# duyhominhnguyen/conan-fgw

Hardware: AMD Instinct MI355X
Metric: molecules/s (K=5 conformers) (higher is better)
Workload: dtype f32

## Files before the change

### conan-fgw_amd/_lib.py

```python
from __future__ import annotations

import ctypes
import os
import subprocess

import torch

_HERE = os.path.dirname(os.path.abspath(__file__))
_SO = os.path.join(_HERE, "libconan_fgw_hip.so")
_LIB = None
ABI_VERSION = 6

c_int, c_float, c_void_p, c_ll = ctypes.c_int, ctypes.c_float, ctypes.c_void_p, ctypes.c_longlong


class FgwParams(ctypes.Structure):
    _fields_ = [("alpha", c_float), ("epsilon", c_float), ("max_iter", c_int), ("tol", c_float), ("inner_tol", c_float),
                ("num_iter_max", c_int), ("stop_thr", c_float), ("fixed_structure", c_int), ("fixed_features", c_int),
                ("warmstart", c_int), ("loss_fun", c_int), ("cs_small_int", c_int)]


class BatchLayout(ctypes.Structure):
    _fields_ = [(n, c_int) for n in ("B", "K", "num_graphs", "num_atoms", "num_bond_edges", "max_nodes", "x_dim", "ea_dim")] + \
               [(n, c_ll) for n in ("off_atom_off", "off_bond_off", "off_z", "off_pos", "off_x", "off_bsrc", "off_bdst", "off_battr", "off_y", "bytes")]


class WgradJob(ctypes.Structure):
    _fields_ = [("ws", c_void_p), ("dW", c_void_p), ("dbias", c_void_p), ("M", c_int), ("K", c_int), ("N", c_int), ("slices", c_int)]


class WgradSlabJob(ctypes.Structure):
    _fields_ = [("g", c_void_p), ("x", c_void_p), ("m_dev", c_void_p), ("ws", c_void_p), ("M", c_int), ("K", c_int), ("N", c_int), ("slices", c_int)]


_P = c_void_p
SIGNATURES = {
    "conan_abi_version": (c_int, []),
    "conan_collate_layout": (c_int, [c_int, c_int, _P, _P, c_int, c_int, ctypes.POINTER(BatchLayout)]),
    "conan_collate_pack": (c_int, [ctypes.POINTER(BatchLayout), _P, _P, _P, _P, _P, _P, _P, _P, _P]),
    "conan_collate_unpack": (c_int, [_P, ctypes.POINTER(BatchLayout), _P, _P, _P, _P, _P, _P, _P, _P, _P, _P, _P]),
    "conan_graph_ptr_from_batch": (c_int, [_P, c_int, c_int, _P, _P]),
    "conan_radius_graph_csr": (c_int, [_P, _P, c_int, c_int, c_float, c_int, c_int, _P, _P, _P, _P, _P, _P]),
    "conan_csr_transpose": (c_int, [_P, c_int, c_int, _P, _P, _P, _P, _P, _P]),
    "conan_edge_pairs": (c_int, [_P, _P, _P, _P, _P, c_int, _P, _P, _P, _P, _P, _P, _P, _P]),
    "conan_edge_index_i64": (c_int, [_P, _P, c_int, _P, _P]),
    "conan_embedding_fwd": (c_int, [_P, _P, c_int, c_int, c_int, _P, _P]),
    "conan_onehot_rows": (c_int, [_P, c_int, c_int, c_int, _P, _P]),
    "conan_embedding_bwd_ws": (c_ll, [c_int, c_int, c_int]),
    "conan_embedding_bwd": (c_int, [_P, _P, c_int, c_int, c_int, c_int, _P, _P, _P]),
    "conan_linear_fwd": (c_int, [_P, _P, _P, _P, c_int, c_int, c_int, c_int, c_int, _P, _P, _P]),
    "conan_linear_multi_fwd": (c_int, [_P, _P, _P, c_int, c_int, c_int, c_int, c_int, _P, _P, _P, _P]),
    "conan_linear_sum_fwd": (c_int, [_P, _P, _P, c_int, c_int, _P, _P, c_int, c_int, _P, _P, _P]),
    "conan_ssp_bwd": (c_int, [_P, _P, c_int, c_int, _P, _P, _P]),
    "conan_linear_wgrad_ws": (c_ll, [c_int, c_int, c_int]),
    "conan_linear_wgrad": (c_int, [_P, _P, c_int, c_int, c_int, _P, _P, _P, _P, _P]),
    "conan_bond_graph_csr": (c_int, [_P, c_int, c_int, _P, _P, _P, _P, _P, _P, _P, _P]),
    "conan_gat_edge_vec": (c_int, [_P, _P, c_int, c_int, _P, _P]),
    "conan_gat_edge_vec_bwd": (c_int, [_P, _P, _P, c_int, c_int, _P, _P, _P]),
    "conan_gat_node_alpha": (c_int, [_P, _P, _P, c_int, c_int, _P, _P, _P]),
    "conan_gat_aggregate_fwd": (c_int, [_P, _P, _P, _P, _P, _P, _P, c_int, _P, _P, c_float, c_int, c_int, _P, _P, _P, _P]),
    "conan_gat_bwd_ws": (c_ll, [c_int, c_int, c_int, c_int]),
    "conan_gat_aggregate_bwd": (c_int, [_P] * 15 + [c_int, _P, c_float, c_int, c_int, c_int, _P, _P, _P, _P]),
    "conan_linear_act_fwd": (c_int, [_P, _P, _P, c_int, c_int, c_int, c_int, _P, _P, _P, _P]),
    "conan_unary_fwd": (c_int, [_P, c_ll, c_int, _P, _P]),
    "conan_unary_bwd": (c_int, [_P, _P, c_ll, c_int, _P, _P]),
    "conan_zero_tail": (c_int, [_P, _P, c_int, c_int, _P]),
    "conan_rbf_wgrad": (c_int, [_P, _P, c_int, _P, c_int, c_float, c_int, _P, _P, _P, _P, _P]),
    "conan_wgrad_batchable": (c_int, [c_int, c_int]),
    "conan_linear_wgrad_scaled": (c_int, [_P, _P, c_int, c_int, c_int, _P, _P, _P, _P, _P, _P]),
    "conan_linear_wgrad_slabs": (c_int, [_P, _P, c_int, c_int, c_int, _P, _P, _P]),
    "conan_rbf_wgrad_slabs": (c_int, [_P, _P, c_int, _P, c_int, c_float, c_int, _P, _P, _P]),
    "conan_wgrad_reduce_batch": (c_int, [ctypes.POINTER(WgradJob), c_int, _P]),
    "conan_linear_wgrad_slabs_batch": (c_int, [ctypes.POINTER(WgradSlabJob), c_int, _P]),
    "conan_filter_bwd_supported": (c_int, [c_int, c_int]),
    "conan_filter_bwd_slices": (c_int, [c_int]),
    "conan_filter_bwd_ws": (c_ll, [c_int, c_int, c_int]),
    "conan_filter_bwd": (c_int, [_P, _P, _P, c_int, _P, c_int, c_float, _P, c_int, _P, _P, _P, _P, _P, _P]),
# ... 160 lines not shown
```

### conan-fgw_amd/csrc/graph.hip

```cpp
#include "common.h"

namespace {

__global__ void k_graph_ptr(const int64_t *__restrict__ batch, int n, int G, int *__restrict__ ptr) {
    int i = blockIdx.x * blockDim.x + threadIdx.x;
    if (i >= n) return;
    long long cur = batch[i];
    long long prev = i == 0 ? -1 : batch[i - 1];
    for (long long g = prev + 1; g <= cur && g < G; ++g) ptr[g] = i;
    if (i == n - 1)
        for (long long g = cur + 1; g <= G; ++g) ptr[g] = n;
}
__global__ void k_graph_ptr_empty(int G, int *ptr) {
    int g = blockIdx.x * blockDim.x + threadIdx.x;
    if (g <= G) ptr[g] = 0;
}

__device__ __forceinline__ float dist2_rn(float ax, float ay, float az, float bx, float by, float bz) {
    float dx = __fsub_rn(ax, bx), dy = __fsub_rn(ay, by), dz = __fsub_rn(az, bz);
    return __fadd_rn(__fadd_rn(__fmul_rn(dx, dx), __fmul_rn(dy, dy)), __fmul_rn(dz, dz));
}

constexpr int RG_THREADS = 128;
constexpr int RG_MAX_LDS_ATOMS = 2048;
// ... 38 lines not shown
constexpr int SCAN_LDS_MAX = 36 * 1024;
__global__ void __launch_bounds__(1024) k_exclusive_scan_lds(const int *__restrict__ in, int n, int *__restrict__ out) {
    extern __shared__ int sdat[];
    int *wsum = sdat + n;
    const int t = threadIdx.x, lane = t & 63, wave = t >> 6;
    for (int i0 = t; i0 < n; i0 += 4 * 1024) {
        int v[4];
#pragma unroll
        for (int u = 0; u < 4; ++u) { const int i = i0 + u * 1024; v[u] = in[i < n ? i : n - 1]; }
#pragma unroll
        for (int u = 0; u < 4; ++u) { const int i = i0 + u * 1024; if (i < n) sdat[i] = v[u]; }
    }
    __syncthreads();
    const int chunk = ((n + 1023) / 1024) | 1;
    const int b = min(t * chunk, n), e = min(b + chunk, n);
    int s = 0;
    for (int i = b; i < e; ++i) s += sdat[i];
    int inc = s;
#pragma unroll
    for (int o = 1; o < 64; o <<= 1) { const int u = __shfl_up(inc, o, 64); if (lane >= o) inc += u; }
    if (lane == 63) wsum[wave] = inc;
    __syncthreads();
    int woff = 0, total = 0;
#pragma unroll
    for (int w = 0; w < 16; ++w) { const int x = wsum[w]; if (w < wave) woff += x; total += x; }
    int run = woff + inc - s;
    for (int i = b; i < e; ++i) { const int x = sdat[i]; sdat[i] = run; run += x; }
    __syncthreads();
    for (int i = t; i < n; i += 1024) out[i] = sdat[i];
    if (t == 0) out[n] = total;
}

constexpr int SCAN_THREADS = 1024;
__global__ void __launch_bounds__(SCAN_THREADS) k_exclusive_scan(const int *__restrict__ in, int n, int *__restrict__ out) {
    __shared__ int wsum[SCAN_THREADS / 64];
    const int t = threadIdx.x, lane = t & 63, wave = t >> 6;
    const int chunk = (n + SCAN_THREADS - 1) / SCAN_THREADS;
    const int b = t * chunk, e = min(b + chunk, n);
    constexpr int MAXC = 32;
    int v[MAXC];
    int s = 0;
    if (chunk <= MAXC) {
#pragma unroll
        for (int k = 0; k < MAXC; ++k) { v[k] = (b + k < e) ? in[b + k] : 0; }
#pragma unroll
        for (int k = 0; k < MAXC; ++k) s += v[k];
    } else {
        for (int i = b; i < e; ++i) s += in[i];
    }
    int inc = s;
#pragma unroll
    for (int o = 1; o < 64; o <<= 1) { const int u = __shfl_up(inc, o, 64); if (lane >= o) inc += u; }
    if (lane == 63) wsum[wave] = inc;
    __syncthreads();
    int woff = 0, total = 0;
#pragma unroll
    for (int w = 0; w < SCAN_THREADS / 64; ++w) { const int x = wsum[w]; if (w < wave) woff += x; total += x; }
    int run = woff + inc - s;
    if (chunk <= MAXC) {
#pragma unroll
        for (int k = 0; k < MAXC; ++k) if (b + k < e) { out[b + k] = run; run += v[k]; }
    } else {
        for (int i = b; i < e; ++i) { const int x = in[i]; out[i] = run; run += x; }
    }
    if (t == 0) out[n] = total;
}

static void launch_exclusive_scan(const int *in, int n, int *out, hipStream_t s) {
    if (n > 0 && n <= SCAN_LDS_MAX) {
        const size_t lds = (size_t)(n + 16) * sizeof(int);
        if (lds > 64 * 1024)
            (void)hipFuncSetAttribute(reinterpret_cast<const void *>(&k_exclusive_scan_lds), hipFuncAttributeMaxDynamicSharedMemorySize, (int)lds);
        k_exclusive_scan_lds<<<1, 1024, lds, s>>>(in, n, out);
    } else {
        k_exclusive_scan<<<1, SCAN_THREADS, 0, s>>>(in, n, out);
    }
}

constexpr int SB_THREADS = 256;
constexpr int SB_ITEMS = 16;
__global__ void __launch_bounds__(SB_THREADS) k_scan_block_sums(const int *__restrict__ in, int n, int *__restrict__ bsum) {
    __shared__ int red[SB_THREADS / 64];
    const int base = blockIdx.x * SB_THREADS * SB_ITEMS + threadIdx.x * SB_ITEMS;
    int s = 0;
#pragma unroll
    for (int u = 0; u < SB_ITEMS; ++u) s += (base + u < n) ? in[base + u] : 0;
    s = wave_sum(s);
    if ((threadIdx.x & 63) == 0) red[threadIdx.x >> 6] = s;
    __syncthreads();
    if (threadIdx.x == 0) bsum[blockIdx.x] = red[0] + red[1] + red[2] + red[3];
}
__global__ void __launch_bounds__(SB_THREADS) k_scan_block_apply(const int *__restrict__ in, int n, const int *__restrict__ boff,
                                                                 int nblocks, int *__restrict__ out) {
    __shared__ int part[SB_THREADS];
    const int t = threadIdx.x;
    const int base = blockIdx.x * SB_THREADS * SB_ITEMS + t * SB_ITEMS;
    int v[SB_ITEMS], s = 0;
#pragma unroll
    for (int u = 0; u < SB_ITEMS; ++u) { v[u] = (base + u < n) ? in[base + u] : 0; s += v[u]; }
    part[t] = s;
    __syncthreads();
    for (int o = 1; o < SB_THREADS; o <<= 1) {
        const int a = t >= o ? part[t - o] : 0;
        __syncthreads();
        part[t] += a;
        __syncthreads();
    }
    int run = boff[blockIdx.x] + (t == 0 ? 0 : part[t - 1]);
#pragma unroll
    for (int u = 0; u < SB_ITEMS; ++u) { if (base + u < n) out[base + u] = run; run += v[u]; }
    if (blockIdx.x == nblocks - 1 && t == SB_THREADS - 1) out[n] = boff[nblocks];
}
static void scan_large(const int *in, int n, int *out, int *ws, hipStream_t s) {
    const int per = SB_THREADS * SB_ITEMS;
    const int nblocks = (n + per - 1) / per;
    int *bsum = ws, *boff = ws + nblocks + 1;
    k_scan_block_sums<<<nblocks, SB_THREADS, 0, s>>>(in, n, bsum);
    launch_exclusive_scan(bsum, nblocks, boff, s);
    k_scan_block_apply<<<nblocks, SB_THREADS, 0, s>>>(in, n, boff, nblocks, out);
}

constexpr int TR_THREADS = 1024;
__global__ void __launch_bounds__(TR_THREADS) k_transpose_graph(const int *__restrict__ gptr, const int *__restrict__ rowptr,
                                                                const int *__restrict__ col, int num_atoms,
                                                                int *__restrict__ t_rowptr, int *__restrict__ t_eid) {
    const int g = blockIdx.x;
    const int lo = gptr[g], hi = gptr[g + 1];
    if (g == gridDim.x - 1 && threadIdx.x == 0) t_rowptr[num_atoms] = rowptr[num_atoms];
    if (hi <= lo) return;
    const int e0 = rowptr[lo], e1 = rowptr[hi];
    const int steps = (e1 - e0 + 63) >> 6;
    const int lane = threadIdx.x & 63, wave = threadIdx.x >> 6;
    const unsigned long long below = (1ull << lane) - 1ull;
    constexpr int TR_REG = 18;
    if (steps <= TR_REG) {
        int cv[TR_REG];
#pragma unroll
        for (int s = 0; s < TR_REG; ++s) {
            const int e = e0 + s * 64 + lane;
            cv[s] = (s < steps && e < e1) ? col[e] : 0x7fffffff;
        }
        for (int j = lo + wave; j < hi; j += TR_THREADS / 64) {
            int less = 0;
#pragma unroll
            for (int s = 0; s < TR_REG; ++s) less += __popcll(__ballot(cv[s] < j));
            int base = e0 + less;
            if (lane == 0) t_rowptr[j] = base;
#pragma unroll
            for (int s = 0; s < TR_REG; ++s) {
                const bool hit = cv[s] == j;
                const unsigned long long m = __ballot(hit);
                if (hit) t_eid[base + __popcll(m & below)] = e0 + s * 64 + lane;
                base += __popcll(m);
            }
        }
        return;
    }
    constexpr int TR_LDS = 4096;
    __shared__ int sc[TR_LDS];
    if (steps * 64 <= TR_LDS) {
        for (int q = threadIdx.x; q < steps * 64; q += TR_THREADS) sc[q] = (e0 + q < e1) ? col[e0 + q] : 0x7fffffff;
        __syncthreads();
        for (int j = lo + wave; j < hi; j += TR_THREADS / 64) {
            int less = 0;
            for (int s = 0; s < steps; ++s) less += __popcll(__ballot(sc[s * 64 + lane] < j));
            int base = e0 + less;
            if (lane == 0) t_rowptr[j] = base;
            for (int s = 0; s < steps; ++s) {
                const bool hit = sc[s * 64 + lane] == j;
                const unsigned long long m = __ballot(hit);
                if (hit) t_eid[base + __popcll(m & below)] = e0 + s * 64 + lane;
                base += __popcll(m);
            }
        }
        return;
    }
    for (int j = lo + wave; j < hi; j += TR_THREADS / 64) {
        int less = 0;
        for (int s = 0; s < steps; ++s) {
            const int e = e0 + s * 64 + lane;
            less += __popcll(__ballot(e < e1 && col[e] < j));
        }
        int base = e0 + less;
        if (lane == 0) t_rowptr[j] = base;
        for (int s = 0; s < steps; ++s) {
            const int e = e0 + s * 64 + lane;
            const bool hit = e < e1 && col[e] == j;
            const unsigned long long m = __ballot(hit);
            if (hit) t_eid[base + __popcll(m & below)] = e;
            base += __popcll(m);
        }
    }
}

__device__ __forceinline__ int find_edge(const int *__restrict__ rowptr, const int *__restrict__ col, int target, int source) {
    int lo = rowptr[target], hi = rowptr[target + 1] - 1;
    while (lo <= hi) {
        const int mid = (lo + hi) >> 1;
        const int c = col[mid];
        if (c == source) return mid;
        if (c < source) lo = mid + 1; else hi = mid - 1;
    }
    return -1;
}
__global__ void k_pair_flag(const int *__restrict__ rowptr, const int *__restrict__ col, const int *__restrict__ tgt,
                            const int *__restrict__ ne_dev, int max_edges, int *__restrict__ flag) {
    const int E = min(*ne_dev, max_edges);
    for (int e = blockIdx.x * blockDim.x + threadIdx.x; e < max_edges; e += gridDim.x * blockDim.x) {
        int f = 0;
        if (e < E) {
            const int s = col[e], t = tgt[e];
            f = (s <= t) ? 1 : (find_edge(rowptr, col, s, t) < 0 ? 1 : 0);
        }
        flag[e] = f;
    }
}
__global__ void k_pair_fill(const int *__restrict__ rowptr, const int *__restrict__ col, const int *__restrict__ tgt, const float *__restrict__ dist,
                            const int *__restrict__ ne_dev, int max_edges, const int *__restrict__ flag, const int *__restrict__ pidx,
                            int *__restrict__ pid, int *__restrict__ pe0, int *__restrict__ pe1, float *__restrict__ pdist) {
    const int E = min(*ne_dev, max_edges);
    for (int e = blockIdx.x * blockDim.x + threadIdx.x; e < E; e += gridDim.x * blockDim.x) {
        const int s = col[e], t = tgt[e];
        const int rev = (s == t) ? -1 : find_edge(rowptr, col, s, t);
        if (flag[e]) {
            const int p = pidx[e];
            pid[e] = p; pe0[p] = e; pe1[p] = rev; pdist[p] = dist[e];
        } else {
            pid[e] = pidx[rev];
        }
    }
}

__global__ void k_edge_index(const int *__restrict__ col, const int *__restrict__ tgt, int E, int64_t *__restrict__ ei) {
    int e = blockIdx.x * blockDim.x + threadIdx.x;
    if (e < E) { ei[e] = col[e]; ei[(size_t)E + e] = tgt[e]; }
}


__global__ void k_bond_count(const int64_t *__restrict__ ei, int E, int n, int *__restrict__ deg_t, int *__restrict__ deg_s) {
    for (int e = blockIdx.x * blockDim.x + threadIdx.x; e < E; e += gridDim.x * blockDim.x) {
        const int s = (int)ei[e], t = (int)ei[(size_t)E + e];
        if (s == t || s < 0 || t < 0 || s >= n || t >= n) continue;
        atomicAdd(&deg_t[t], 1);
        atomicAdd(&deg_s[s], 1);
    }
}
__global__ void k_bond_fill_t(const int64_t *__restrict__ ei, int E, int n, const int *__restrict__ rowptr, int *__restrict__ cursor,
                              int *__restrict__ col, int *__restrict__ eid) {
    for (int e = blockIdx.x * blockDim.x + threadIdx.x; e < E; e += gridDim.x * blockDim.x) {
        const int s = (int)ei[e], t = (int)ei[(size_t)E + e];
        if (s == t || s < 0 || t < 0 || s >= n || t >= n) continue;
        const int p = rowptr[t] + atomicAdd(&cursor[t], 1);
        col[p] = s; eid[p] = e;
    }
}
__global__ void k_rows_sort2(const int *__restrict__ rowptr, int n, int *__restrict__ key, int *__restrict__ val) {
    for (int i = blockIdx.x * blockDim.x + threadIdx.x; i < n; i += gridDim.x * blockDim.x) {
        const int a = rowptr[i], b = rowptr[i + 1];
        for (int p = a + 1; p < b; ++p) {
            const int k = key[p], v = val[p];
            int q = p - 1;
            while (q >= a && (key[q] > k || (key[q] == k && val[q] > v))) { key[q + 1] = key[q]; val[q + 1] = val[q]; --q; }
            key[q + 1] = k; val[q + 1] = v;
        }
    }
// ... 30 lines not shown
                           int loop, int *deg_ws, int *rowptr, int *col, int *tgt, float *dist, void *stream) {
    if (!pos || !graph_ptr || !deg_ws || !rowptr || !col || !tgt || !dist || num_atoms < 0 || num_graphs <= 0 || cap <= 0)
        return CONAN_E_BADARG;
    hipStream_t s = as_stream(stream);
    const float r2 = r * r;
    k_radius<0><<<num_graphs, RG_THREADS, 0, s>>>(pos, graph_ptr, r2, cap, loop, deg_ws, nullptr, nullptr, nullptr, nullptr);
    launch_exclusive_scan(deg_ws, num_atoms, rowptr, s);
    k_radius<1><<<num_graphs, RG_THREADS, 0, s>>>(pos, graph_ptr, r2, cap, loop, nullptr, rowptr, col, tgt, dist);
    CONAN_LAUNCH_CHECK();
    return CONAN_OK;
}

int conan_csr_transpose(const int *graph_ptr, int num_graphs, int num_atoms, const int *rowptr, const int *col,
                        int *deg_ws, int *t_rowptr, int *t_eid, void *stream) {
    if (!graph_ptr || !rowptr || !col || !t_rowptr || !t_eid || num_graphs <= 0) return CONAN_E_BADARG;
    hipStream_t s = as_stream(stream);
    (void)deg_ws;
    k_transpose_graph<<<num_graphs, TR_THREADS, 0, s>>>(graph_ptr, rowptr, col, num_atoms, t_rowptr, t_eid);
    CONAN_LAUNCH_CHECK();
    return CONAN_OK;
}

int conan_edge_pairs(const int *rowptr, const int *col, const int *tgt, const float *dist, const int *num_edges_dev, int max_edges,
                     int *flag_ws, int *pidx_ws, int *scan_ws, int *pid, int *pair_e0, int *pair_e1, float *pair_dist, void *stream) {
    if (!rowptr || !col || !tgt || !dist || !num_edges_dev || !flag_ws || !pidx_ws || !scan_ws || !pid || !pair_e0 || !pair_e1 || !pair_dist ||
        max_edges <= 0)
        return CONAN_E_BADARG;
    hipStream_t s = as_stream(stream);
    int blocks = (max_edges + 255) / 256;
    if (blocks > 4096) blocks = 4096;
    k_pair_flag<<<blocks, 256, 0, s>>>(rowptr, col, tgt, num_edges_dev, max_edges, flag_ws);
    scan_large(flag_ws, max_edges, pidx_ws, scan_ws, s);
    k_pair_fill<<<blocks, 256, 0, s>>>(rowptr, col, tgt, dist, num_edges_dev, max_edges, flag_ws, pidx_ws, pid, pair_e0, pair_e1, pair_dist);
    CONAN_LAUNCH_CHECK();
    return CONAN_OK;
}

int conan_bond_graph_csr(const int64_t *edge_index, int num_edges, int num_nodes, int *ws, int *rowptr, int *col, int *eid,
                         int *t_rowptr, int *t_pos, int *t_tgt, void *stream) {
    if (num_edges < 0 || num_nodes <= 0 || !ws || !rowptr || !t_rowptr || (num_edges && (!edge_index || !col || !eid || !t_pos || !t_tgt)))
        return CONAN_E_BADARG;
    hipStream_t s = as_stream(stream);
    int *deg_t = ws, *deg_s = ws + (num_nodes + 1);
    if (hipMemsetAsync(ws, 0, sizeof(int) * 2 * (size_t)(num_nodes + 1), s) != hipSuccess) return CONAN_E_LAUNCH;
    const int eb = num_edges ? (num_edges + 255) / 256 : 1, nb = (num_nodes + 255) / 256;
    if (num_edges) k_bond_count<<<eb, 256, 0, s>>>(edge_index, num_edges, num_nodes, deg_t, deg_s);
    launch_exclusive_scan(deg_t, num_nodes, rowptr, s);
    launch_exclusive_scan(deg_s, num_nodes, t_rowptr, s);
    if (num_edges) {
        if (hipMemsetAsync(ws, 0, sizeof(int) * 2 * (size_t)(num_nodes + 1), s) != hipSuccess) return CONAN_E_LAUNCH;
        k_bond_fill_t<<<eb, 256, 0, s>>>(edge_index, num_edges, num_nodes, rowptr, deg_t, col, eid);
        k_rows_sort2<<<nb, 256, 0, s>>>(rowptr, num_nodes, col, eid);
        k_bond_fill_s<<<nb, 256, 0, s>>>(rowptr, col, num_nodes, t_rowptr, deg_s, t_pos, t_tgt);
        k_rows_sort2<<<nb, 256, 0, s>>>(t_rowptr, num_nodes, t_pos, t_tgt);
    }
    CONAN_LAUNCH_CHECK();
    return CONAN_OK;
}

int conan_edge_index_i64(const int *col, const int *tgt, int num_edges, int64_t *edge_index, void *stream) {
    if (num_edges < 0 || (num_edges && (!col || !tgt || !edge_index))) return CONAN_E_BADARG;
    if (num_edges == 0) return CONAN_OK;
    k_edge_index<<<(num_edges + 255) / 256, 256, 0, as_stream(stream)>>>(col, tgt, num_edges, edge_index);
    CONAN_LAUNCH_CHECK();
    return CONAN_OK;
}
// ... 3 lines not shown
```

### conan-fgw_amd/ops.py

```python
from __future__ import annotations

import ctypes
from typing import Optional

import torch
from torch import Tensor

from ._lib import FgwParams, call, lib, ptr, stream_ptr

f32, i32, i64 = torch.float32, torch.int32, torch.int64


def _c(t: Tensor) -> Tensor:
    return t if t.is_contiguous() else t.contiguous()


class RadiusGraph:

    def __init__(self, pos: Tensor, graph_ptr: Tensor, num_graphs: int, cutoff: float, max_num_neighbors: int, loop: bool = False):
        pos = _c(pos)
        if pos.dtype != f32:
            raise RuntimeError("pos must be float32")
        n = pos.shape[0]
        dev = pos.device
        self.num_atoms, self.num_graphs, self.graph_ptr = n, num_graphs, graph_ptr
        self.cutoff, self.cap, self.loop = float(cutoff), int(max_num_neighbors), bool(loop)
        self.max_edges = max(1, n * (self.cap if self.loop else self.cap + 1))
        self.rowptr = torch.empty(n + 1, dtype=i32, device=dev)
        self.col = torch.empty(self.max_edges, dtype=i32, device=dev)
        self.tgt = torch.empty(self.max_edges, dtype=i32, device=dev)
        self.dist = torch.empty(self.max_edges, dtype=f32, device=dev)
        self._deg = torch.empty(n + 1, dtype=i32, device=dev)
        call("conan_radius_graph_csr", ptr(pos), ptr(graph_ptr, i32), n, num_graphs, self.cutoff, self.cap, int(self.loop),
             ptr(self._deg), ptr(self.rowptr), ptr(self.col), ptr(self.tgt), ptr(self.dist), stream_ptr())
        self.num_edges_dev = self.rowptr[n:]
        self._num_edges: Optional[int] = None
        self._t_rowptr = self._t_eid = None
        self.pid = None

    @property
    def num_edges(self) -> int:
        if self._num_edges is None:
            self._num_edges = int(self.num_edges_dev.item())
        return self._num_edges

    def transpose(self):
        if self._t_rowptr is None:
            dev = self.rowptr.device
            self._t_rowptr = torch.empty(self.num_atoms + 1, dtype=i32, device=dev)
            self._t_eid = torch.empty(self.max_edges, dtype=i32, device=dev)
            call("conan_csr_transpose", ptr(self.graph_ptr), self.num_graphs, self.num_atoms, ptr(self.rowptr), ptr(self.col),
                 ptr(self._deg), ptr(self._t_rowptr), ptr(self._t_eid), stream_ptr())
        return self._t_rowptr, self._t_eid

    def pairs(self):
        if getattr(self, "pid", None) is None:
            dev, ME = self.rowptr.device, self.max_edges
            flag = torch.empty(ME + 1, dtype=i32, device=dev)
            pidx = torch.empty(ME + 1, dtype=i32, device=dev)
            scan_ws = torch.empty(2 * (ME // 4096 + 2), dtype=i32, device=dev)
            self.pid = torch.empty(ME, dtype=i32, device=dev)
            self.pair_e0 = torch.empty(ME, dtype=i32, device=dev)
            self.pair_e1 = torch.empty(ME, dtype=i32, device=dev)
            self.pair_dist = torch.empty(ME, dtype=f32, device=dev)
            call("conan_edge_pairs", ptr(self.rowptr), ptr(self.col), ptr(self.tgt), ptr(self.dist), ptr(self.num_edges_dev), ME, ptr(flag),
                 ptr(pidx), ptr(scan_ws), ptr(self.pid), ptr(self.pair_e0), ptr(self.pair_e1), ptr(self.pair_dist), stream_ptr())
            self.num_pairs_dev = pidx[ME:]
        return self

    def edge_index(self) -> Tensor:
        E = self.num_edges
# ... 1146 lines not shown
```

### conan-fgw_amd/schnet.py

```python
from __future__ import annotations

import math
from typing import Callable, Optional

import torch
from torch import Tensor
from torch.nn import Embedding, Linear, ModuleList, Sequential

from . import ops

OptTensor = Optional[Tensor]


class ShiftedSoftplus(torch.nn.Module):

    def __init__(self):
        super().__init__()
        self.shift = math.log(2.0)

    def forward(self, x: Tensor) -> Tensor:
        return ops.shifted_softplus(x)


class GaussianSmearing(torch.nn.Module):
    def __init__(self, start: float = 0.0, stop: float = 5.0, num_gaussians: int = 50):
        super().__init__()
        offset = torch.linspace(start, stop, num_gaussians)
        self.coeff = -0.5 / (offset[1] - offset[0]).item() ** 2
        self.register_buffer("offset", offset)

    def forward(self, graph: ops.RadiusGraph) -> Tensor:
        return ops.rbf_expand(graph, self.offset, self.coeff)


class RadiusInteractionGraph(torch.nn.Module):

    def __init__(self, cutoff: float = 10.0, max_num_neighbors: int = 32):
        super().__init__()
        self.cutoff = cutoff
        self.max_num_neighbors = max_num_neighbors

    def csr(self, pos: Tensor, graph_ptr: Tensor, num_graphs: int) -> ops.RadiusGraph:
        return ops.RadiusGraph(pos, graph_ptr, num_graphs, self.cutoff, self.max_num_neighbors, loop=False)

    def forward(self, pos: Tensor, batch: Tensor):
        num_graphs = int(batch[-1].item()) + 1 if batch.numel() else 0
        g = self.csr(pos, ops.graph_ptr_from_batch(batch, num_graphs), num_graphs)
        return g.edge_index(), g.edge_weight()


FUSE_FILTER_INTO_GATHER = True
FUSE_MIN_FILTER_BYTES = 192 << 20


def _filter_tensor_outgrows_cache(graph: "ops.RadiusGraph", num_filters: int) -> bool:
    n, G = graph.num_atoms, max(1, graph.num_graphs)
    est_pairs = 0.5 * n * min(float(graph.cap), max(0.0, n / G - 1.0))
    return est_pairs * num_filters * 4 >= FUSE_MIN_FILTER_BYTES

class CFConv(torch.nn.Module):
    def __init__(self, in_channels: int, out_channels: int, num_filters: int, nn: Sequential, cutoff: float):
        super().__init__()
        self.lin1 = Linear(in_channels, num_filters, bias=False)
        self.lin2 = Linear(num_filters, out_channels)
        self.nn = nn
        self.cutoff = cutoff
        self.reset_parameters()

    def reset_parameters(self):
        torch.nn.init.xavier_uniform_(self.lin1.weight)
        torch.nn.init.xavier_uniform_(self.lin2.weight)
        self.lin2.bias.data.fill_(0)

    def forward(self, x: Tensor, graph: ops.RadiusGraph, rbf, tap: bool = False):
        if isinstance(rbf, Tensor):
            md = graph.num_edges_dev
# ... 62 lines not shown
        self.device = device
        self.hidden_channels = hidden_channels
        self.num_filters = num_filters
        self.num_interactions = num_interactions
        self.num_gaussians = num_gaussians
        self.cutoff = cutoff
        self.use_readout = use_readout
        self.use_covalent = use_covalent
        self.fused_filter = True
        self.mean, self.std, self.scale = mean, std, None
        self.embedding = Embedding(100, hidden_channels, padding_idx=0)
        self.interaction_graph = RadiusInteractionGraph(cutoff, max_num_neighbors)
        self.distance_expansion = GaussianSmearing(0.0, cutoff, num_gaussians)
        self.interactions = ModuleList([InteractionBlock(hidden_channels, num_gaussians, num_filters, cutoff)
                                        for _ in range(num_interactions)])
        self.lin1 = Linear(hidden_channels, hidden_channels // 2)
        self.act = ShiftedSoftplus()
        self.register_buffer("initial_atomref", None)
        self.atomref = None
        torch.nn.init.xavier_uniform_(self.lin1.weight)
        self.lin1.bias.data.fill_(0)
        self.lin1_bary = Linear(hidden_channels, hidden_channels // 2)
        self.lin2_bary = Linear(hidden_channels // 2, hidden_channels // 2)
        self.lin2 = Linear(hidden_channels // 2, hidden_channels // 2)

    def _graphs(self, z: Tensor, pos: Tensor, batch: OptTensor, num_graphs: Optional[int]):
        if not z.is_cuda:
            raise RuntimeError("SchNetNoSum (MI355X) runs on the GPU only: move the inputs to the device; there is no CPU fallback")
        batch = torch.zeros_like(z) if batch is None else batch
        hint_g, hint_n = ops.batch_hints(batch)
        if num_graphs is None:
            num_graphs = hint_g if hint_g is not None else int(batch[-1].item()) + 1
        gptr = ops.graph_ptr_from_batch(batch, num_graphs)
        graph = self.interaction_graph.csr(pos, gptr, num_graphs)
        graph.max_nodes_hint = hint_n if hint_g == num_graphs else None
        return batch, gptr, graph, num_graphs

    def _trunk(self, z: Tensor, graph: ops.RadiusGraph) -> Tensor:
        h = ops.embedding(z, self.embedding.weight, self.embedding.padding_idx)
        if self.fused_filter and ops.filter_fused_supported(self.num_gaussians, self.num_filters):
            rbf = (self.distance_expansion.offset, self.distance_expansion.coeff)
        else:
            rbf = self.distance_expansion(graph)
        for interaction in self.interactions:
            h = interaction(h, graph, rbf)
        return h

    def _head(self, h: Tensor, lin1: Linear, lin2: Linear) -> Tensor:
        return ops.mlp2_outact(h, lin1.weight, lin1.bias, lin2.weight, lin2.bias)

    def forward(self, z: Tensor, pos: Tensor, batch: OptTensor = None, data_batch=None, num_graphs: Optional[int] = None) -> Tensor:
        batch, gptr, graph, G = self._graphs(z, pos, batch, num_graphs)
        h = self._head(self._trunk(z, graph), self.lin1, self.lin2)
        return ops.segment_sum(h, gptr, G) if self.use_readout else h

    def forward_3d_bary(self, z: Tensor, pos: Tensor, batch: OptTensor = None, data_batch=None, num_graphs: Optional[int] = None,
                        _graph=None):
        if _graph is None:
            _, _, graph, _ = self._graphs(z, pos, batch, num_graphs)
        else:
            graph = _graph
        h_shared = self._trunk(z, graph)
        h = self._head(h_shared, self.lin1, self.lin2)
        h_bary = self._head(h_shared, self.lin1_bary, self.lin2_bary)
        return h, h_bary

    def _compute_barycenter(self, node_feature: Tensor, edge_index, batch: Tensor, batch_size: int, num_conformers: int,
# ... 54 lines not shown
```

### conan-fgw_amd/visnet.py

```python
from __future__ import annotations

import math
from typing import Optional

import torch
from torch import Tensor
from torch.nn import Embedding, LayerNorm, Linear

from . import ops
from . import visnet_ops as vo
from ._lib import call, ptr, stream_ptr

f32 = torch.float32


class ExpNormalSmearing(torch.nn.Module):
    def __init__(self, cutoff: float = 5.0, num_rbf: int = 32):
        super().__init__()
        self.cutoff, self.num_rbf, self.alpha = cutoff, num_rbf, 5.0 / cutoff
        start = torch.exp(torch.tensor(-cutoff))
        self.register_buffer("means", torch.linspace(start, 1, num_rbf))
        self.register_buffer("betas", torch.tensor([(2 / num_rbf * (1 - start)) ** -2] * num_rbf))


# ... 36 lines not shown
        self.layernorm = LayerNorm(hidden)
        self.vec_layernorm = VecLayerNorm(hidden)
        self.vec_proj = Linear(hidden, hidden * 3, False)
        self.q_proj, self.k_proj, self.v_proj = Linear(hidden, hidden), Linear(hidden, hidden), Linear(hidden, hidden)
        self.dk_proj, self.dv_proj = Linear(hidden, hidden), Linear(hidden, hidden)
        self.s_proj = Linear(hidden, hidden * 2)
        if not last_layer:
            self.f_proj = Linear(hidden, hidden)
            self.w_src_proj = Linear(hidden, hidden, False)
            self.w_trg_proj = Linear(hidden, hidden, False)
        self.o_proj = Linear(hidden, hidden * 3)
        for m in self.modules():
            if isinstance(m, Linear):
                torch.nn.init.xavier_uniform_(m.weight)
                if m.bias is not None:
                    m.bias.data.zero_()


class ViSNetBlock(torch.nn.Module):
    def __init__(self, num_heads=8, num_layers=6, hidden_channels=128, num_rbf=32, max_z=100, cutoff=5.0, max_num_neighbors=32):
        super().__init__()
        self.num_heads, self.hidden_channels, self.cutoff, self.max_num_neighbors = num_heads, hidden_channels, cutoff, max_num_neighbors
        self.embedding = Embedding(max_z, hidden_channels)
        self.distance_expansion = ExpNormalSmearing(cutoff, num_rbf)
        self.neighbor_embedding = NeighborEmbedding(hidden_channels, num_rbf, cutoff, max_z)
        self.edge_embedding = EdgeEmbedding(num_rbf, hidden_channels)
        self.vis_mp_layers = torch.nn.ModuleList([ViS_MP(num_heads, hidden_channels, cutoff, last_layer=(i == num_layers - 1))
                                                  for i in range(num_layers)])
        self.out_norm = LayerNorm(hidden_channels)
        self.vec_out_norm = VecLayerNorm(hidden_channels)

    def forward(self, z: Tensor, pos: Tensor, graph_ptr: Tensor, num_graphs: int):
        H, dev, n, s = self.hidden_channels, z.device, z.shape[0], stream_ptr()
        g = ops.RadiusGraph(pos, graph_ptr, num_graphs, self.cutoff, self.max_num_neighbors, loop=True)
        md, ME = g.num_edges_dev, g.max_edges
        dvec = torch.empty(ME, 3, dtype=f32, device=dev)
        call("conan_visnet_edge_unit", ptr(pos.contiguous(), f32), ptr(g.col), ptr(g.tgt), ptr(md), ME, ptr(dvec), s)
        de = self.distance_expansion
        rbf = ops.empty_rows(ME, de.num_rbf, dev, md)
        call("conan_visnet_expnormal", ptr(g.dist), ptr(md), ME, ptr(de.means), ptr(de.betas), de.num_rbf, de.alpha, de.cutoff, ptr(rbf), s)
        x = ops.embedding(z, self.embedding.weight, None)
        ne = self.neighbor_embedding
        W = vo.neighbor_scale(vo.lin(rbf, ne.distance_proj, False, md), g, self.cutoff)
        xn = ops.cfconv(ops.embedding(z, ne.embedding.weight, None), W, g)
        x = vo.lin(vo.concat2(x, xn), ne.combine)
        vec = torch.zeros(n, 3, H, dtype=f32, device=dev)
        f = vo.edge_embed(x, vo.lin(rbf, self.edge_embedding.edge_proj, False, md), g)
        on_side = False
        for layer in self.vis_mp_layers:
            x, vec, f, on_side = self._vis_mp(layer, x, vec, f, g, dvec, on_side)
        return vo.layernorm(x, self.out_norm), vo.scale_channels(vec, self.vec_out_norm.weight)

    def _vis_mp(self, L: ViS_MP, x, vec, f, g, dvec, inputs_on_side: bool = False):
        H, n = self.hidden_channels, x.shape[0]
        md = g.num_edges_dev
        wt = ws = None
        x_res = x
        vec_res = vec

        def node_level():
            nonlocal wt, ws, vec_res, x_res
            if TAP_X_RESIDUAL:
                xl_, x_res = vo.layernorm(x, L.layernorm, tap=True)
            else:
                xl_ = vo.layernorm(x, L.layernorm)
            if TAP_VEC_RESIDUAL:
                vl_, vec_res = vo.scale_channels(vec, L.vec_layernorm.weight, tap=True)
# ... 183 lines not shown
```

### include/conan_fgw_hip.h

```cpp
#ifndef CONAN_FGW_HIP_H
#define CONAN_FGW_HIP_H

#include <stdint.h>

#ifdef __cplusplus
extern "C" {
#endif

#define CONAN_OK 0
#define CONAN_E_BADARG (-1)
#define CONAN_E_LAUNCH (-2)
#define CONAN_E_UNSUPPORTED (-3)

#define CONAN_FGW_ABI_VERSION 6
int conan_abi_version(void);


typedef struct conan_batch_layout {
    int B, K;
    int num_graphs;
    int num_atoms;
    int num_bond_edges;
    int max_nodes;
    int x_dim, ea_dim;
    long long off_atom_off, off_bond_off;
    long long off_z;
    long long off_pos;
    long long off_x;
    long long off_bsrc, off_bdst;
    long long off_battr;
    long long off_y;
    long long bytes;
} conan_batch_layout;

int conan_collate_layout(int B, int K, const int *n_atoms, const int *n_bonds, int x_dim, int ea_dim, conan_batch_layout *layout);
int conan_collate_pack(const conan_batch_layout *layout, const int *n_atoms, const int *n_bonds, const int64_t *const *z,
                       const float *const *pos, const float *const *x, const int64_t *const *edge_index,
                       const float *const *edge_attr, const float *y, void *packed);
int conan_collate_unpack(const void *packed_dev, const conan_batch_layout *layout, int64_t *z, float *pos, int64_t *batch,
                         float *x, int64_t *edge_index, float *edge_attr, float *y, int *graph_ptr, int64_t *conformers_index,
                         int64_t *conf_node_batch, void *stream);


int conan_graph_ptr_from_batch(const int64_t *batch, int num_atoms, int num_graphs, int *graph_ptr, void *stream);

int conan_radius_graph_csr(const float *pos, const int *graph_ptr, int num_atoms, int num_graphs, float r, int cap,
                           int loop, int *deg_ws, int *rowptr, int *col, int *tgt, float *dist, void *stream);

int conan_csr_transpose(const int *graph_ptr, int num_graphs, int num_atoms, const int *rowptr, const int *col,
                        int *deg_ws, int *t_rowptr, int *t_eid, void *stream);

int conan_edge_pairs(const int *rowptr, const int *col, const int *tgt, const float *dist, const int *num_edges_dev,
                     int max_edges, int *flag_ws, int *pidx_ws, int *scan_ws, int *pid, int *pair_e0, int *pair_e1,
                     float *pair_dist, void *stream);

int conan_edge_index_i64(const int *col, const int *tgt, int num_edges, int64_t *edge_index, void *stream);


int conan_embedding_fwd(const int64_t *z, const float *weight, int num_atoms, int hidden, int num_embeddings, float *out,
                        void *stream);
int conan_onehot_rows(const int64_t *z, int num_atoms, int num_embeddings, int padding_idx, float *out, void *stream);
long long conan_embedding_bwd_ws(int num_atoms, int hidden, int num_embeddings);
int conan_embedding_bwd(const int64_t *z, const float *dout, int num_atoms, int hidden, int num_embeddings,
                        int padding_idx, float *dweight, float *ws, void *stream);

int conan_linear_fwd(const float *x, const float *w, const float *bias, const float *residual, int M, int K, int N,
                     int w_kn, int act, const int *m_dev, float *y, void *stream);

int conan_linear_act_fwd(const float *x, const float *w, const float *bias, int M, int K, int N, int act, const int *m_dev,
                         float *y, float *pre, void *stream);

int conan_linear_multi_fwd(const float *x, const float *const *w, const float *const *bias, int M, int K, int N, int num_layers, int act,
                           const int *m_dev, float *const *y, float *const *pre, void *stream);
int conan_linear_sum_fwd(const float *const *x, const int *ldx, const float *const *w, int num_inputs, int w_kn, const float *bias,
                         const float *residual, int M, int N, const int *m_dev, float *y, void *stream);
int conan_ssp_bwd(const float *dy, const float *y, int rows, int width, const int *m_dev, float *g, void *stream);
long long conan_linear_wgrad_ws(int M, int K, int N);
int conan_linear_wgrad(const float *g, const float *x, int M, int K, int N, const int *m_dev, float *dW, float *dbias,
                       float *ws, void *stream);
int conan_linear_wgrad_scaled(const float *g, const float *x, int M, int K, int N, const int *m_dev, float *dW, float *dbias, float *ws,
                              const float *gmax, void *stream);
int conan_rbf_wgrad(const float *g, const float *dist, int M, const float *offset, int num_gaussians, float coeff, int N,
                    const int *m_dev, float *dW, float *dbias, float *ws, void *stream);

typedef struct conan_wgrad_job {
    const float *ws;
    float *dW, *dbias;
// ... 242 lines not shown
```

Before: 116,000.

## Fuse radius graph, edge pairs and CSR transpose into per-graph build kernels

Replaces the separate radius-graph CSR, edge-pair flagging/scan/fill and CSR transpose launches with a three-kernel build. One per-graph kernel computes neighbor lists in LDS, reverse-edge indices and pair ranks. A combined two-array scan follows, then a per-graph fill kernel writes CSR, pairs and the transpose, using reverse indices directly when the graph is symmetric. The goal is fewer launches and global-memory passes over edges. The cost is a larger workspace and more complex code.

```diff
diff --git a/conan-fgw_amd/_lib.py b/conan-fgw_amd/_lib.py
--- a/conan-fgw_amd/_lib.py
+++ b/conan-fgw_amd/_lib.py
@@ -43,6 +43,8 @@
     "conan_radius_graph_csr": (c_int, [_P, _P, c_int, c_int, c_float, c_int, c_int, _P, _P, _P, _P, _P, _P]),
     "conan_csr_transpose": (c_int, [_P, c_int, c_int, _P, _P, _P, _P, _P, _P]),
     "conan_edge_pairs": (c_int, [_P, _P, _P, _P, _P, c_int, _P, _P, _P, _P, _P, _P, _P, _P]),
+    "conan_radius_graph_build_ws": (c_ll, [c_int, c_int, c_int, c_int]),
+    "conan_radius_graph_build": (c_int, [_P, _P, c_int, c_int, c_float, c_int, c_int] + [_P] * 12 + [_P]),
     "conan_edge_index_i64": (c_int, [_P, _P, c_int, _P, _P]),
     "conan_embedding_fwd": (c_int, [_P, _P, c_int, c_int, c_int, _P, _P]),
     "conan_onehot_rows": (c_int, [_P, c_int, c_int, c_int, _P, _P]),
diff --git a/conan-fgw_amd/csrc/graph.hip b/conan-fgw_amd/csrc/graph.hip
--- a/conan-fgw_amd/csrc/graph.hip
+++ b/conan-fgw_amd/csrc/graph.hip
@@ -94,7 +94,7 @@
 }
 
 constexpr int SCAN_THREADS = 1024;
-__global__ void __launch_bounds__(SCAN_THREADS) k_exclusive_scan(const int *__restrict__ in, int n, int *__restrict__ out) {
+__device__ __forceinline__ void exclusive_scan_block(const int *__restrict__ in, int n, int *__restrict__ out) {
     __shared__ int wsum[SCAN_THREADS / 64];
     const int t = threadIdx.x, lane = t & 63, wave = t >> 6;
     const int chunk = (n + SCAN_THREADS - 1) / SCAN_THREADS;
@@ -127,6 +127,14 @@
     }
     if (t == 0) out[n] = total;
 }
+__global__ void __launch_bounds__(SCAN_THREADS) k_exclusive_scan(const int *__restrict__ in, int n, int *__restrict__ out) {
+    exclusive_scan_block(in, n, out);
+}
+__global__ void __launch_bounds__(SCAN_THREADS) k_exclusive_scan_two(const int *__restrict__ in0, const int *__restrict__ in1, int n,
+                                                                     int *__restrict__ out0, int *__restrict__ out1) {
+    if (blockIdx.x == 0) exclusive_scan_block(in0, n, out0);
+    else exclusive_scan_block(in1, n, out1);
+}
 
 static void launch_exclusive_scan(const int *in, int n, int *out, hipStream_t s) {
     if (n > 0 && n <= SCAN_LDS_MAX) {
@@ -183,14 +191,8 @@
 }
 
 constexpr int TR_THREADS = 1024;
-__global__ void __launch_bounds__(TR_THREADS) k_transpose_graph(const int *__restrict__ gptr, const int *__restrict__ rowptr,
-                                                                const int *__restrict__ col, int num_atoms,
-                                                                int *__restrict__ t_rowptr, int *__restrict__ t_eid) {
-    const int g = blockIdx.x;
-    const int lo = gptr[g], hi = gptr[g + 1];
-    if (g == gridDim.x - 1 && threadIdx.x == 0) t_rowptr[num_atoms] = rowptr[num_atoms];
-    if (hi <= lo) return;
-    const int e0 = rowptr[lo], e1 = rowptr[hi];
+__device__ __forceinline__ void transpose_graph_rows(int lo, int hi, int e0, int e1, const int *__restrict__ col,
+                                                     int *__restrict__ t_rowptr, int *__restrict__ t_eid) {
     const int steps = (e1 - e0 + 63) >> 6;
     const int lane = threadIdx.x & 63, wave = threadIdx.x >> 6;
     const unsigned long long below = (1ull << lane) - 1ull;
@@ -254,6 +256,15 @@
         }
     }
 }
+__global__ void __launch_bounds__(TR_THREADS) k_transpose_graph(const int *__restrict__ gptr, const int *__restrict__ rowptr,
+                                                                const int *__restrict__ col, int num_atoms,
+                                                                int *__restrict__ t_rowptr, int *__restrict__ t_eid) {
+    const int g = blockIdx.x;
+    const int lo = gptr[g], hi = gptr[g + 1];
+    if (g == gridDim.x - 1 && threadIdx.x == 0) t_rowptr[num_atoms] = rowptr[num_atoms];
+    if (hi <= lo) return;
+    transpose_graph_rows(lo, hi, rowptr[lo], rowptr[hi], col, t_rowptr, t_eid);
+}
 
 __device__ __forceinline__ int find_edge(const int *__restrict__ rowptr, const int *__restrict__ col, int target, int source) {
     int lo = rowptr[target], hi = rowptr[target + 1] - 1;
@@ -293,6 +304,203 @@
     }
 }
 
+constexpr int GB_THREADS = 256;
+constexpr int GB_POS_LDS = 1024;
+constexpr int GB_LIST_LDS = 4096;
+struct GraphBuildWs {
+    int *deg, *lrow, *prow;
+    int *ecnt, *pcnt, *eoff, *poff;
+    int *sym;
+    int *s_col, *s_rev, *s_rank;
+    float *s_dist;
+};
+static long long graph_build_ws_ints(long long n, long long G, long long W) { return 3 * n + 5 * G + 2 + 4 * n * W; }
+static GraphBuildWs graph_build_ws(int *ws, int n, int G, int W) {
+    GraphBuildWs w;
+    const size_t nw = (size_t)n * W;
+    w.deg = ws; w.lrow = w.deg + n; w.prow = w.lrow + n;
+    w.ecnt = w.prow + n; w.pcnt = w.ecnt + G; w.eoff = w.pcnt + G; w.poff = w.eoff + G + 1; w.sym = w.poff + G + 1;
+    w.s_col = w.sym + G; w.s_rev = w.s_col + nw; w.s_rank = w.s_rev + nw;
+    w.s_dist = reinterpret_cast<float *>(w.s_rank + nw);
+    return w;
+}
+
+template <int NT>
+__device__ __forceinline__ int block_exclusive_scan(const int *in, int n, int *out, int *wsum) {
+    const int t = threadIdx.x, lane = t & 63, wave = t >> 6;
+    int carry = 0;
+    for (int base = 0; base < n; base += NT) {
+        const int i = base + t;
+        const int v = i < n ? in[i] : 0;
+        int inc = v;
+#pragma unroll
+        for (int o = 1; o < 64; o <<= 1) { const int u = __shfl_up(inc, o, 64); if (lane >= o) inc += u; }
+        if (lane == 63) wsum[wave] = inc;
+        __syncthreads();
+        int woff = 0, total = 0;
+#pragma unroll
+        for (int w = 0; w < NT / 64; ++w) { const int x = wsum[w]; if (w < wave) woff += x; total += x; }
+        if (i < n) out[i] = carry + woff + inc - v;
+        carry += total;
+        __syncthreads();
+    }
+    return carry;
+}
+
+template <bool LDS>
+__device__ __forceinline__ void graph_build_local(int g, int n, int W, int want_pairs, const short *s_col, short *s_rev, const short *s_deg,
+                                                  const int *gcol, int *grev, int *grank, const int *gdeg, int *prow, int *wsum,
+                                                  const GraphBuildWs &ws) {
+    auto col_at = [&](int idx) { return LDS ? (int)s_col[idx] : gcol[idx]; };
+    auto deg_at = [&](int i) { return LDS ? (int)s_deg[i] : gdeg[i]; };
+    int missing = 0;
+    for (int idx = threadIdx.x; idx < n * W; idx += GB_THREADS) {
+        const int i = idx / W, k = idx - i * W;
+        if (k >= deg_at(i)) continue;
+        const int s = col_at(idx);
+        int a = 0, b = deg_at(s) - 1, rev = -1;
+        while (a <= b) {
+            const int mid = (a + b) >> 1;
+            const int c = col_at(s * W + mid);
+            if (c == i) { rev = mid; break; }
+            if (c < i) a = mid + 1; else b = mid - 1;
+        }
+        grev[idx] = rev;
+        if (LDS) s_rev[idx] = (short)rev;
+        missing |= rev < 0;
+    }
+    __threadfence_block();
+    const int any_missing = __syncthreads_or(missing);
+    if (threadIdx.x == 0) ws.sym[g] = any_missing ? 0 : 1;
+    if (!want_pairs) {
+        if (threadIdx.x == 0) ws.pcnt[g] = 0;
+        return;
+    }
+    for (int i = threadIdx.x; i < n; i += GB_THREADS) {
+        const int d = deg_at(i);
+        int cnt = 0;
+        for (int k = 0; k < d; ++k) {
+            const int idx = i * W + k;
+            const int rev = LDS ? (int)s_rev[idx] : grev[idx];
+            const bool rep = col_at(idx) <= i || rev < 0;
+            grank[idx] = rep ? cnt : -1;
+            cnt += rep;
+        }
+        prow[i] = cnt;
+    }
+    __threadfence_block();
+    __syncthreads();
+    const int np = block_exclusive_scan<GB_THREADS>(prow, n, prow, wsum);
+    if (threadIdx.x == 0) ws.pcnt[g] = np;
+}
+
+__global__ void __launch_bounds__(GB_THREADS) k_graph_build_lists(const float *__restrict__ pos, const int *__restrict__ gptr, float r2, int cap,
+                                                                  int loop, int W, int want_rev, int want_pairs, GraphBuildWs ws) {
+    __shared__ float sp[GB_POS_LDS * 3];
+    __shared__ short s_col[GB_LIST_LDS], s_rev[GB_LIST_LDS], s_deg[GB_POS_LDS];
+    __shared__ int wsum[GB_THREADS / 64];
+    const int g = blockIdx.x;
+    const int lo = gptr[g], hi = gptr[g + 1];
+    const int n = hi - lo;
+    if (n <= 0) {
+        if (threadIdx.x == 0) { ws.ecnt[g] = 0; ws.pcnt[g] = 0; ws.sym[g] = 0; }
+        return;
+    }
+    const bool in_lds = n <= GB_POS_LDS;
+    const bool list_lds = in_lds && n * W <= GB_LIST_LDS;
+    const size_t slice = (size_t)lo * W;
+    int *gcol = ws.s_col + slice, *grev = ws.s_rev + slice, *grank = ws.s_rank + slice;
+    float *gdist = ws.s_dist + slice;
+    int *deg = ws.deg + lo;
+    if (in_lds)
+        for (int t = threadIdx.x; t < n * 3; t += GB_THREADS) sp[t] = pos[(size_t)lo * 3 + t];
+    __syncthreads();
+    for (int i = threadIdx.x; i < n; i += GB_THREADS) {
+        float ax, ay, az;
+        if (in_lds) { ax = sp[i * 3]; ay = sp[i * 3 + 1]; az = sp[i * 3 + 2]; }
+        else { ax = pos[(size_t)(lo + i) * 3]; ay = pos[(size_t)(lo + i) * 3 + 1]; az = pos[(size_t)(lo + i) * 3 + 2]; }
+        const int limit = loop ? cap : cap + 1;
+        int cnt = 0, out = 0;
+        for (int j = 0; j < n && cnt < limit; ++j) {
+            float bx, by, bz;
+            if (in_lds) { bx = sp[j * 3]; by = sp[j * 3 + 1]; bz = sp[j * 3 + 2]; }
+            else { bx = pos[(size_t)(lo + j) * 3]; by = pos[(size_t)(lo + j) * 3 + 1]; bz = pos[(size_t)(lo + j) * 3 + 2]; }
+            const float d2 = dist2_rn(bx, by, bz, ax, ay, az);
+            if (d2 < r2) {
+                ++cnt;
+                if (loop || j != i) {
+                    gcol[i * W + out] = j; gdist[i * W + out] = __fsqrt_rn(d2);
+                    if (list_lds) s_col[i * W + out] = (short)j;
+                    ++out;
+                }
+            }
+        }
+        deg[i] = out;
+        if (list_lds) s_deg[i] = (short)out;
+    }
+    __threadfence_block();
+    __syncthreads();
+    const int ne = block_exclusive_scan<GB_THREADS>(deg, n, ws.lrow + lo, wsum);
+    if (threadIdx.x == 0) ws.ecnt[g] = ne;
+    if (!want_rev) {
+        if (threadIdx.x == 0) { ws.pcnt[g] = 0; ws.sym[g] = 0; }
+        return;
+    }
+    if (list_lds) graph_build_local<true>(g, n, W, want_pairs, s_col, s_rev, s_deg, gcol, grev, grank, deg, ws.prow + lo, wsum, ws);
+    else graph_build_local<false>(g, n, W, want_pairs, s_col, s_rev, s_deg, gcol, grev, grank, deg, ws.prow + lo, wsum, ws);
+}
+
+__global__ void __launch_bounds__(TR_THREADS) k_graph_build_fill(const int *__restrict__ gptr, int num_atoms, int W, GraphBuildWs ws,
+                                                                 int *__restrict__ rowptr, int *col, int *__restrict__ tgt,
+                                                                 float *__restrict__ dist, int *__restrict__ pid, int *__restrict__ pe0,
+                                                                 int *__restrict__ pe1, float *__restrict__ pdist, int *__restrict__ num_pairs,
+                                                                 int *__restrict__ t_rowptr, int *__restrict__ t_eid) {
+    const int g = blockIdx.x, G = gridDim.x;
+    const int lo = gptr[g], hi = gptr[g + 1];
+    const int n = hi - lo;
+    if (g == G - 1 && threadIdx.x == 0) {
+        const int E = ws.eoff[G];
+        rowptr[num_atoms] = E;
+        if (t_rowptr) t_rowptr[num_atoms] = E;
+        if (num_pairs) *num_pairs = ws.poff[G];
+    }
+    if (n <= 0) return;
+    const int eo = ws.eoff[g], po = ws.poff[g];
+    const bool sym = t_eid && ws.sym[g];
+    const size_t slice = (size_t)lo * W;
+    const int *gcol = ws.s_col + slice, *grev = ws.s_rev + slice, *grank = ws.s_rank + slice;
+    const float *gdist = ws.s_dist + slice;
+    const int *deg = ws.deg + lo, *lrow = ws.lrow + lo, *prow = ws.prow + lo;
+    for (int i = threadIdx.x; i < n; i += TR_THREADS) {
+        const int r = eo + lrow[i];
+        rowptr[lo + i] = r;
+        if (sym) t_rowptr[lo + i] = r;
+    }
+    for (int idx = threadIdx.x; idx < n * W; idx += TR_THREADS) {
+        const int i = idx / W, k = idx - i * W;
+        if (k >= deg[i]) continue;
+        const int e = eo + lrow[i] + k;
+        const int s = gcol[idx];
+        const float d = gdist[idx];
+        col[e] = lo + s; tgt[e] = lo + i; dist[e] = d;
+        if (pid) {
+            const int rev = grev[idx], rk = grank[idx];
+            if (rk >= 0) {
+                const int p = po + prow[i] + rk;
+                pid[e] = p; pe0[p] = e; pe1[p] = (s == i || rev < 0) ? -1 : eo + lrow[s] + rev; pdist[p] = d;
+            } else {
+                pid[e] = po + prow[s] + grank[s * W + rev];
+            }
+        }
+        if (sym) t_eid[e] = eo + lrow[s] + grev[idx];
+    }
+    if (t_eid && !sym) {
+        __threadfence_block();
+        __syncthreads();
+        transpose_graph_rows(lo, hi, eo, eo + ws.ecnt[g], col, t_rowptr, t_eid);
+    }
+}
+
 __global__ void k_edge_index(const int *__restrict__ col, const int *__restrict__ tgt, int E, int64_t *__restrict__ ei) {
     int e = blockIdx.x * blockDim.x + threadIdx.x;
     if (e < E) { ei[e] = col[e]; ei[(size_t)E + e] = tgt[e]; }
@@ -389,6 +597,31 @@
     k_pair_flag<<<blocks, 256, 0, s>>>(rowptr, col, tgt, num_edges_dev, max_edges, flag_ws);
     scan_large(flag_ws, max_edges, pidx_ws, scan_ws, s);
     k_pair_fill<<<blocks, 256, 0, s>>>(rowptr, col, tgt, dist, num_edges_dev, max_edges, flag_ws, pidx_ws, pid, pair_e0, pair_e1, pair_dist);
+    CONAN_LAUNCH_CHECK();
+    return CONAN_OK;
+}
+
+long long conan_radius_graph_build_ws(int num_atoms, int num_graphs, int cap, int loop) {
+    if (num_atoms < 0 || num_graphs < 0 || cap <= 0) return CONAN_E_BADARG;
+    return graph_build_ws_ints(num_atoms, num_graphs, loop ? cap : cap + 1);
+}
+
+int conan_radius_graph_build(const float *pos, const int *graph_ptr, int num_atoms, int num_graphs, float r, int cap, int loop, int *ws,
+                             int *rowptr, int *col, int *tgt, float *dist, int *pid, int *pair_e0, int *pair_e1, float *pair_dist,
+                             int *num_pairs, int *t_rowptr, int *t_eid, void *stream) {
+    if ((!pos && num_atoms > 0) || !graph_ptr || !ws || !rowptr || !col || !tgt || !dist || num_atoms < 0 || num_graphs <= 0 || cap <= 0)
+        return CONAN_E_BADARG;
+    const bool pairs = pid || pair_e0 || pair_e1 || pair_dist || num_pairs;
+    if (pairs && !(pid && pair_e0 && pair_e1 && pair_dist && num_pairs)) return CONAN_E_BADARG;
+    if ((t_rowptr == nullptr) != (t_eid == nullptr)) return CONAN_E_BADARG;
+    const int W = loop ? cap : cap + 1;
+    if ((long long)num_atoms * W > 0x7fffffffLL) return CONAN_E_UNSUPPORTED;
+    hipStream_t s = as_stream(stream);
+    const GraphBuildWs w = graph_build_ws(ws, num_atoms, num_graphs, W);
+    k_graph_build_lists<<<num_graphs, GB_THREADS, 0, s>>>(pos, graph_ptr, r * r, cap, loop, W, pairs || t_eid, pairs, w);
+    k_exclusive_scan_two<<<2, SCAN_THREADS, 0, s>>>(w.ecnt, w.pcnt, num_graphs, w.eoff, w.poff);
+    k_graph_build_fill<<<num_graphs, TR_THREADS, 0, s>>>(graph_ptr, num_atoms, W, w, rowptr, col, tgt, dist, pid, pair_e0, pair_e1, pair_dist,
+                                                         num_pairs, t_rowptr, t_eid);
     CONAN_LAUNCH_CHECK();
     return CONAN_OK;
 }
diff --git a/conan-fgw_amd/ops.py b/conan-fgw_amd/ops.py
--- a/conan-fgw_amd/ops.py
+++ b/conan-fgw_amd/ops.py
@@ -15,9 +15,13 @@
     return t if t.is_contiguous() else t.contiguous()
 
 
+FUSED_GRAPH_BUILD = True
+
+
 class RadiusGraph:
 
-    def __init__(self, pos: Tensor, graph_ptr: Tensor, num_graphs: int, cutoff: float, max_num_neighbors: int, loop: bool = False):
+    def __init__(self, pos: Tensor, graph_ptr: Tensor, num_graphs: int, cutoff: float, max_num_neighbors: int, loop: bool = False,
+                 pairs: bool = False, transpose: bool = False):
         pos = _c(pos)
         if pos.dtype != f32:
             raise RuntimeError("pos must be float32")
@@ -25,18 +29,34 @@
         dev = pos.device
         self.num_atoms, self.num_graphs, self.graph_ptr = n, num_graphs, graph_ptr
         self.cutoff, self.cap, self.loop = float(cutoff), int(max_num_neighbors), bool(loop)
-        self.max_edges = max(1, n * (self.cap if self.loop else self.cap + 1))
+        self.max_edges = ME = max(1, n * (self.cap if self.loop else self.cap + 1))
         self.rowptr = torch.empty(n + 1, dtype=i32, device=dev)
-        self.col = torch.empty(self.max_edges, dtype=i32, device=dev)
-        self.tgt = torch.empty(self.max_edges, dtype=i32, device=dev)
-        self.dist = torch.empty(self.max_edges, dtype=f32, device=dev)
+        self.col = torch.empty(ME, dtype=i32, device=dev)
+        self.tgt = torch.empty(ME, dtype=i32, device=dev)
+        self.dist = torch.empty(ME, dtype=f32, device=dev)
         self._deg = torch.empty(n + 1, dtype=i32, device=dev)
-        call("conan_radius_graph_csr", ptr(pos), ptr(graph_ptr, i32), n, num_graphs, self.cutoff, self.cap, int(self.loop),
-             ptr(self._deg), ptr(self.rowptr), ptr(self.col), ptr(self.tgt), ptr(self.dist), stream_ptr())
+        self._t_rowptr = self._t_eid = None
+        self.pid = None
+        if FUSED_GRAPH_BUILD:
+            ws = torch.empty(max(1, lib().conan_radius_graph_build_ws(n, num_graphs, self.cap, int(self.loop))), dtype=i32, device=dev)
+            if pairs:
+                self.pid = torch.empty(ME, dtype=i32, device=dev)
+                self.pair_e0 = torch.empty(ME, dtype=i32, device=dev)
+                self.pair_e1 = torch.empty(ME, dtype=i32, device=dev)
+                self.pair_dist = torch.empty(ME, dtype=f32, device=dev)
+                self.num_pairs_dev = torch.empty(1, dtype=i32, device=dev)
+            if transpose:
+                self._t_rowptr = torch.empty(n + 1, dtype=i32, device=dev)
+                self._t_eid = torch.empty(ME, dtype=i32, device=dev)
+            call("conan_radius_graph_build", ptr(pos) if n else None, ptr(graph_ptr, i32), n, num_graphs, self.cutoff, self.cap, int(self.loop), ptr(ws),
+                 ptr(self.rowptr), ptr(self.col), ptr(self.tgt), ptr(self.dist),
+                 ptr(self.pid), ptr(self.pair_e0 if pairs else None), ptr(self.pair_e1 if pairs else None), ptr(self.pair_dist if pairs else None),
+                 ptr(self.num_pairs_dev if pairs else None), ptr(self._t_rowptr), ptr(self._t_eid), stream_ptr())
+        else:
+            call("conan_radius_graph_csr", ptr(pos), ptr(graph_ptr, i32), n, num_graphs, self.cutoff, self.cap, int(self.loop),
+                 ptr(self._deg), ptr(self.rowptr), ptr(self.col), ptr(self.tgt), ptr(self.dist), stream_ptr())
         self.num_edges_dev = self.rowptr[n:]
         self._num_edges: Optional[int] = None
-        self._t_rowptr = self._t_eid = None
-        self.pid = None
 
     @property
     def num_edges(self) -> int:
diff --git a/conan-fgw_amd/schnet.py b/conan-fgw_amd/schnet.py
--- a/conan-fgw_amd/schnet.py
+++ b/conan-fgw_amd/schnet.py
@@ -40,8 +40,8 @@
         self.cutoff = cutoff
         self.max_num_neighbors = max_num_neighbors
 
-    def csr(self, pos: Tensor, graph_ptr: Tensor, num_graphs: int) -> ops.RadiusGraph:
-        return ops.RadiusGraph(pos, graph_ptr, num_graphs, self.cutoff, self.max_num_neighbors, loop=False)
+    def csr(self, pos: Tensor, graph_ptr: Tensor, num_graphs: int, pairs: bool = False, transpose: bool = False) -> ops.RadiusGraph:
+        return ops.RadiusGraph(pos, graph_ptr, num_graphs, self.cutoff, self.max_num_neighbors, loop=False, pairs=pairs, transpose=transpose)
 
     def forward(self, pos: Tensor, batch: Tensor):
         num_graphs = int(batch[-1].item()) + 1 if batch.numel() else 0
@@ -170,7 +170,8 @@
         if num_graphs is None:
             num_graphs = hint_g if hint_g is not None else int(batch[-1].item()) + 1
         gptr = ops.graph_ptr_from_batch(batch, num_graphs)
-        graph = self.interaction_graph.csr(pos, gptr, num_graphs)
+        pairs = self.fused_filter and ops.filter_fused_supported(self.num_gaussians, self.num_filters)
+        graph = self.interaction_graph.csr(pos, gptr, num_graphs, pairs=pairs, transpose=torch.is_grad_enabled())
         graph.max_nodes_hint = hint_n if hint_g == num_graphs else None
         return batch, gptr, graph, num_graphs
 
diff --git a/conan-fgw_amd/visnet.py b/conan-fgw_amd/visnet.py
--- a/conan-fgw_amd/visnet.py
+++ b/conan-fgw_amd/visnet.py
@@ -92,7 +92,8 @@
 
     def forward(self, z: Tensor, pos: Tensor, graph_ptr: Tensor, num_graphs: int):
         H, dev, n, s = self.hidden_channels, z.device, z.shape[0], stream_ptr()
-        g = ops.RadiusGraph(pos, graph_ptr, num_graphs, self.cutoff, self.max_num_neighbors, loop=True)
+        g = ops.RadiusGraph(pos, graph_ptr, num_graphs, self.cutoff, self.max_num_neighbors, loop=True,
+                            transpose=torch.is_grad_enabled())
         md, ME = g.num_edges_dev, g.max_edges
         dvec = torch.empty(ME, 3, dtype=f32, device=dev)
         call("conan_visnet_edge_unit", ptr(pos.contiguous(), f32), ptr(g.col), ptr(g.tgt), ptr(md), ME, ptr(dvec), s)
diff --git a/include/conan_fgw_hip.h b/include/conan_fgw_hip.h
--- a/include/conan_fgw_hip.h
+++ b/include/conan_fgw_hip.h
@@ -53,6 +53,11 @@
 int conan_edge_pairs(const int *rowptr, const int *col, const int *tgt, const float *dist, const int *num_edges_dev,
                      int max_edges, int *flag_ws, int *pidx_ws, int *scan_ws, int *pid, int *pair_e0, int *pair_e1,
                      float *pair_dist, void *stream);
+
+long long conan_radius_graph_build_ws(int num_atoms, int num_graphs, int cap, int loop);
+int conan_radius_graph_build(const float *pos, const int *graph_ptr, int num_atoms, int num_graphs, float r, int cap, int loop, int *ws,
+                             int *rowptr, int *col, int *tgt, float *dist, int *pid, int *pair_e0, int *pair_e1, float *pair_dist,
+                             int *num_pairs, int *t_rowptr, int *t_eid, void *stream);
 
 int conan_edge_index_i64(const int *col, const int *tgt, int num_edges, int64_t *edge_index, void *stream);
 
```

After: 117,200, median of 6. +1.1%, better.
